# Derek-TH-Wang/OpenRoboRL

Hardware: AMD Instinct MI355X
Metric: env steps/sec at N parallel robots (higher is better)
Workload: dtype f32

## Files before the change

### openroborl_amd/csrc/orr_env_kernels.h

```cpp
#pragma once
#if defined(ORR_PHASE_TIMERS) && !defined(ORR_WAVE_TIMELINE)
#define ORR_WAVE_TIMELINE 1
#endif
#ifndef ORR_TU_MAIN
#undef ORR_PHASE_TIMERS
#endif
#include <hip/hip_runtime.h>
#include <type_traits>
#include <math.h>
#include <stdint.h>
#include <stdio.h>
#include <stdlib.h>
#include <string.h>

#include "orr_device.h"

#ifdef ORR_PHASE_TIMERS
__device__ long long g_phase_cycles[orr::kPhaseSlots];
__device__ long long g_wave_phases[2048 * 40];
#define PT_INIT() do { if (threadIdx.x == 0) { for (int i_ = 0; i_ < orr::kPhaseSlots; i_++) S.pt_acc[i_] = 0; S.pt_last = clock64(); } } while (0)
#define PT(k) do { if (threadIdx.x == 0) { const long long t_ = clock64(); S.pt_acc[k] += t_ - S.pt_last; S.pt_last = clock64(); } } while (0)
#define PT_FLUSH() do { if (threadIdx.x == 0 && blockIdx.x == gridDim.x / 2) for (int i_ = 0; i_ < orr::kPhaseSlots; i_++) atomicAdd((unsigned long long*)&g_phase_cycles[i_], (unsigned long long)S.pt_acc[i_]); \
                        if (threadIdx.x == 0 && blockIdx.x < 2048) for (int i_ = 0; i_ < orr::kPhaseSlots; i_++) g_wave_phases[blockIdx.x * 40 + i_] = S.pt_acc[i_]; } while (0)
#else
// ... 46 lines not shown
  load_robot(P, rec, S, lane);
  const long long total = P.counters[ORR_CNT_TOTAL_STEP_COUNT];
  const ResetConst RC = load_reset_const(P, S, lane);
  float clip_change = 0.0f;
  const uint32_t ep = reset_robot_state<CLIPS, NOISE>(P, S, lane, total, RC, &clip_change, uniforms ? uniforms + (size_t)robot * 28 : nullptr);
  build_obs<NOISE>(P, rec, S, lane, obs, ep, 0u);
  WSYNC();
  store_reset_extras<CLIPS>(rec, S, lane, valid, clip_change);
  store_robot(rec, S, lane, valid);
  if (valid)
    for (int i = lane; i < ORR_OFFEND_ANCHOR_VALID - ORR_OFF_ANCHOR + 1; i += kLanes) rec[O(ANCHOR) + i] = 0.0f;
  if (obs_out && valid)
    for (int i = lane; i < ORR_OBS_DIM; i += kLanes) obs_out[(size_t)robot * ORR_OBS_DIM + i] = obs[i];
}

template <bool CLIPS = true>
__global__ __launch_bounds__(64) void orr_sensor_reset_kernel(KParams P, const uint8_t* mask, float* obs_out, const float* uniforms) {
  ORR_PROLOGUE();
  const bool valid = in_range && !(mask && !mask[robot]);
  load_robot(P, rec, S, lane);
  const long long total = P.counters[ORR_CNT_TOTAL_STEP_COUNT];
  const ResetConst RC = load_reset_const(P, S, lane);
  const SensorNoise SN = load_sensor_noise(P);
  float clip_change = 0.0f;
  const uint32_t ep = reset_robot_state<CLIPS, true, true>(P, S, lane, total, RC, &clip_change, uniforms ? uniforms + (size_t)robot * 28 : nullptr, SN);
  build_obs<true, true>(P, rec, S, lane, obs, ep, 0u, SN);
  WSYNC();
  store_reset_extras<CLIPS>(rec, S, lane, valid, clip_change);
  store_robot(rec, S, lane, valid);
  if (valid)
    for (int i = lane; i < ORR_OFFEND_ANCHOR_VALID - ORR_OFF_ANCHOR + 1; i += kLanes) rec[O(ANCHOR) + i] = 0.0f;
  if (obs_out && valid)
    for (int i = lane; i < ORR_OBS_DIM; i += kLanes) obs_out[(size_t)robot * ORR_OBS_DIM + i] = obs[i];
}

template <bool CLIPS = true>
__global__ __launch_bounds__(64) void orr_randomizer_reset_kernel(KParams P, const uint8_t* mask, float* obs_out, const float* uniforms) {
  ORR_PROLOGUE();
  const bool valid = in_range && !(mask && !mask[robot]);
  load_robot(P, rec, S, lane);
  const long long total = P.counters[ORR_CNT_TOTAL_STEP_COUNT];
  const ResetConst RC = load_reset_const(P, S, lane);
  const SensorNoise SN = load_sensor_noise(P);
  RandRow RR = load_rand_row(P, robot);
  float clip_change = 0.0f;
  const uint32_t ep = reset_robot_state<CLIPS, true, true, true>(P, S, lane, total, RC, &clip_change, uniforms ? uniforms + (size_t)robot * 28 : nullptr, SN, &RR);
  build_obs<true, true>(P, rec, S, lane, obs, ep, 0u, SN);
  WSYNC();
  store_reset_extras<CLIPS>(rec, S, lane, valid, clip_change);
  store_rand_row(P, RR, lane, valid);
  store_robot(rec, S, lane, valid);
  if (valid)
    for (int i = lane; i < ORR_OFFEND_ANCHOR_VALID - ORR_OFF_ANCHOR + 1; i += kLanes) rec[O(ANCHOR) + i] = 0.0f;
  if (obs_out && valid)
    for (int i = lane; i < ORR_OBS_DIM; i += kLanes) obs_out[(size_t)robot * ORR_OBS_DIM + i] = obs[i];
}

#ifndef ORR_WAVES_PER_EU
#define ORR_WAVES_PER_EU 1
#endif
template <int MODE, int WPE = ORR_WAVES_PER_EU, bool ANCHOR = false, bool CLIPS = false, bool NOISE = false>
__global__ __launch_bounds__(64) __attribute__((amdgpu_waves_per_eu(WPE, WPE))) void orr_step_kernel(KParams P, const float* actions, float* obs_out, float* reward_out,
                                                      uint8_t* done_out, int nsub, ReplayArgs RP) {
  constexpr bool TERMS = (MODE & kModeTerms) != 0;
  static_assert(!TERMS || (MODE & 3) != 1, "the debug physics computes no reward");
  constexpr bool CONTACTS = (MODE & kModeContacts) != 0;
  static_assert(!CONTACTS || (MODE & 3) != 2, "the parity replay replaces the physics by recorded states: it has no impulses");
  constexpr bool ACT = (MODE & kModeActuator) != 0;
  static_assert(!ACT || (MODE & 3) != 1, "the debug physics takes its torques as given");
  static_assert(!ACT || TERMS, "the actuator variants are supersets: instantiated with the reward terms only");
  constexpr bool SENS = (MODE & kModeSensor) != 0;
  static_assert(!SENS || (ACT && NOISE), "the sensor variants are supersets: instantiated on top of the actuator variants only");
  constexpr bool RAND = (MODE & kModeRandomizer) != 0;
  static_assert(!RAND || SENS, "the randomiser variants are supersets: instantiated on top of the sensor variants only");
  constexpr bool PUSH = (MODE & kModePush) != 0;
  static_assert(!PUSH || RAND, "the push variant is a superset: instantiated on top of the randomiser variant only");
  static_assert(!PUSH || (MODE & 3) == 0, "the parity replay replaces the physics by recorded states, the debug physics has no env step: neither is pushed");
  ORR_PROLOGUE();
  const bool valid = in_range;
  const orr_config& c = P.cfg;
  PT_INIT();
  WT_INIT();
  const long long total_snapshot = P.counters[ORR_CNT_TOTAL_STEP_COUNT];
  load_robot(P, rec, S, lane);
  bool terms_bound = true, contacts_bound = true, act_bound = false;
  if constexpr (ACT) {
    terms_bound = P.tab->terms != nullptr;
    contacts_bound = P.tab->contact_out != nullptr;
    act_bound = P.tab->act_out != nullptr;
  }
  RandRow RR;
  if constexpr (RAND) RR = load_rand_row(P, robot);
  typedef float __attribute__((address_space(1)))* gpush;
  PushSet PS;
  float push_old = 0.0f, push_w = 0.0f;
  if constexpr (PUSH) {
    PS = load_push(P);
    if (PS.out) push_old = ((gpush)PS.out)[(size_t)robot * ORR_PUSH_ROW + 7];
  }
  float clip_change = 0.0f;
  if constexpr (CLIPS) clip_change = rec[O(CLIP_CHANGE_TIME)];
  {
    static_assert(kHead > ORR_OFF_RING, "spare LDS word behind the state head (the head = everything in front of the ring)");
    bool bad_in = false;
    for (int i = lane; i < 37; i += kLanes) bad_in = bad_in || !(fabsf(S.s[O(POS) + i]) < 1e30f);
    const bool any_bad = ((__ballot(bad_in) >> (sub * kLanes)) & ((1ull << (kLanes - 1)) * 2ull - 1ull)) != 0ull;
    if (lane == 0) S.s[kHead - 1] = any_bad ? 1.0f : 0.0f;
  }
  for (int i = lane; i < kMaxRows * kWStride; i += kLanes) (&S.ph.sub.W[0][0])[i] = 0.0f;
  WSYNC();
  LegConst K;
  load_leg_const(P, S, lane, K);
  {
    float rel[4], Rb[9];
    base_rotation(S, lane, rel, Rb);
  }
  AnchorState AS = {{0.0f, 0.0f, 0.0f}, {0.0f, 0.0f, 0.0f}, 0};
  bool anchor_robot = false;
  const int aleg = lane < 4 ? lane : (lane < 8 ? lane - 4 : (lane - 8) >> 1);
  if constexpr (ANCHOR) {
    static_assert(kLanes == 16, "ANCHOR: aleg indexes the record's four cached points by the 16-lane row layout");
    anchor_robot = model_cold(P, geti(S, O(ROBOT_TYPE)))->friction_anchor != 0;
    const float* an = rec + O(ANCHOR) + 6 * aleg;
    AS.la[0] = an[0]; AS.la[1] = an[1]; AS.la[2] = an[2]; AS.wb[0] = an[3]; AS.wb[1] = an[4]; AS.wb[2] = an[5];
    AS.valid = anchor_robot ? __float_as_int(rec[O(ANCHOR_VALID) + aleg]) : 0;
  }
  auto store_anchor = [&]() __attribute__((always_inline)) {
    if constexpr (ANCHOR) {
      if (valid && lane >= 4 && lane < 8) {
        float* an = rec + O(ANCHOR) + 6 * aleg;
        an[0] = AS.la[0]; an[1] = AS.la[1]; an[2] = AS.la[2]; an[3] = AS.wb[0]; an[4] = AS.wb[1]; an[5] = AS.wb[2];
        rec[O(ANCHOR_VALID) + aleg] = __int_as_float(AS.valid);
      }
    }
  };
  typedef float __attribute__((address_space(1)))* gcontact;
  const int cw = lane < 12 ? lane : 0;
  float c_sum = 0.0f, c_max = 0.0f;
  auto accumulate_contacts = [&]() __attribute__((always_inline)) {
    if constexpr (CONTACTS) {
      const float lw = S.s[O(LAMBDA) + cw];
      c_sum += lw;
      c_max = fmaxf(c_max, lw);
    }
  };
  auto store_contacts = [&]() __attribute__((always_inline)) {
    if constexpr (CONTACTS) {
      if (valid && lane < 12 && contacts_bound) {
        const int cleg = lane / 3, cd = lane - 3 * cleg;
        gcontact const row = (gcontact)P.tab->contact_out + (size_t)robot * 16 + 4 * cleg;
        row[cd] = c_sum;
        if (cd == 0) row[3] = c_max;
      }
    }
  };
  PT(0);

  if ((MODE & 3) == 1) {
    if (lane < 12) {
      const ColdPtr mc = model_cold(P, geti(S, O(ROBOT_TYPE)));
      const int j = mc->joint_of_motor[lane];
      S.tau[j] = mc->tau_sign_motor[lane] * actions[(size_t)robot * 12 + lane];
    }
    WSYNC();
    int fall = 0;
    OwnCoord X;
    load_own_coord(S, lane, X);
    int limit_idle = 0;
    for (int s = 0; s < nsub; s++) {
      fall = physics_substep<ANCHOR>(P, S, K, lane, sub, true, X, limit_idle, ANCHOR ? &AS : nullptr, anchor_robot);
      accumulate_contacts();
      float rel[4], Rb[9];
      base_rotation(S, lane, rel, Rb);
      WSYNC();
    }
    if (valid && lane == 0 && done_out) done_out[robot] = (uint8_t)fall;
    store_robot(rec, S, lane, valid);
    store_anchor();
    store_contacts();
    return;
  }

  const int ml = lane < 12 ? lane : 0;
  const ColdPtr mc = model_cold(P, geti(S, O(ROBOT_TYPE)));
  const int mj = mc->joint_of_motor[ml];
  const float m_off = mc->motor_offset[ml], m_dir = mc->motor_dir[ml], m_kp = mc->kp[ml], m_kd = mc->kd[ml];
  const float m_tsign = mc->tau_sign_motor[ml], m_init = mc->init_motor_angles[ml];
  typedef float __attribute__((address_space(1)))* gact;
  float a_lim = INFINITY, a_tau = 0.0f, a_s1 = 0.0f, a_pk = 0.0f, a_s2 = 0.0f, a_w = 0.0f;
  if constexpr (ACT) a_lim = ((const float __attribute__((address_space(1)))*)&P.tab->torque_limit[geti(S, O(ROBOT_TYPE))][0])[ml];
  SensorNoise SN;
  uint32_t sn_robot = 0u, sn_ep = 0u, sn_i = 0u;
  if constexpr (SENS) {
    SN = load_sensor_noise(P);
    sn_robot = (uint32_t)geti(S, O(ROBOT_INDEX)); sn_ep = (uint32_t)geti(S, O(EPISODE_IDX)); sn_i = 1u + (uint32_t)geti(S, O(EP_STEP));
  }
  ctrl_obs(P, rec, S, lane);
  float act_in = actions[(size_t)robot * 12 + ml];
  {
    const bool bad_act = !(fabsf(act_in) < 1e30f);
    if (bad_act) act_in = 0.0f;
    const bool any_bad = ((__ballot(bad_act) >> (sub * kLanes)) & ((1ull << (kLanes - 1)) * 2ull - 1ull)) != 0ull;
    if (lane == 0 && any_bad) S.s[kHead - 1] = 1.0f;
  }
  if (lane < 12) {
    const float act = act_in + m_init;
    S.s[O(LAST_ACTION) + lane] = act;
    float x1 = S.s[O(XHIST) + lane], x2 = S.s[O(XHIST) + 12 + lane], y1 = S.s[O(YHIST) + lane], y2 = S.s[O(YHIST) + 12 + lane];
    if (geti(S, O(STATE_ACTION_COUNTER)) == 0) {
      float d = map_pi(S.co[lane]);
      if constexpr (SENS) {
        if (SN.a > 0.0f) {
          float u4[4], z0, z1;
          philox_block(c.seed, sn_robot, sn_ep, sensor_block(sn_i, kSensorSlotFilter, (uint32_t)lane), u4);
          normal_pair(u4[0], u4[1], &z0, &z1);
          d = map_pi(fmaf(SN.a, z0, S.co[lane]));
        }
      }
      x1 = x2 = y1 = y2 = d;
    }
    const float y = act * P.fb[0] + (x1 * P.fb[1] + x2 * P.fb[2]) - (y1 * P.fa[1] + y2 * P.fa[2]);
    S.s[O(XHIST) + 12 + lane] = x1; S.s[O(XHIST) + lane] = act;
    S.s[O(YHIST) + 12 + lane] = y1; S.s[O(YHIST) + lane] = y;
    S.s[O(ACTION) + lane] = y;
  }
  if constexpr (PUSH) {
    static_assert(ORR_OFF_ANGVEL == ORR_OFF_LINVEL + 3, "LINVEL and ANGVEL are six consecutive words");
    const uint32_t ps = sn_i - 1u;
    float ua[4], ub[4] = {0.5f, 0.5f, 0.5f, 0.5f};
    philox_block(c.seed, sn_robot, sn_ep, kPushBlock + 2u * ps, ua);
    const bool kicked = (int)ps >= PS.grace && ua[0] < PS.prob;
    float sn, cs;
    unit_sincos(ua[1], &sn, &cs);
    const float pm = fmaf(ua[2], PS.span, PS.lin_lo);
    if (PS.ang > 0.0f) philox_block(c.seed, sn_robot, sn_ep, kPushBlock + 2u * ps + 1u, ub);
    const float two_ang = PS.ang > 0.0f ? 2.0f * PS.ang : 0.0f;
    const float mine = lane == 0 ? __fmul_rn(pm, cs) : (lane == 1 ? __fmul_rn(pm, sn) : (lane == 2 ? fmaf(ua[3], 2.0f * PS.lin_z, -PS.lin_z)
                       : fmaf(lane == 3 ? ub[0] : (lane == 4 ? ub[1] : ub[2]), two_ang, -PS.ang)));
    const float dk = kicked && lane < 6 ? mine : 0.0f;
    if (lane < 6) {
      const float v = S.s[O(LINVEL) + lane];
      S.s[O(LINVEL) + lane] = kicked ? __fadd_rn(v, dk) : v;
    }
    const float one = kicked ? 1.0f : 0.0f;
    push_w = lane < 6 ? dk : (lane == 6 ? one : (ps == 0u ? 0.0f : push_old) + one);
  }
  WSYNC();
  PT(1);
  int fall = 0;
  const float inv_repeat = 1.0f / (float)c.action_repeat;
  const RingLatency rlat = ring_latency(P, S);
  const float m_gain = m_tsign * S.s[O(STRENGTH) + ml];
  const float m_target = S.s[O(ACTION) + ml], m_prev = S.s[O(FILTER_ACTION) + ml];
  const bool m_has_prev = geti(S, O(FILTER_VALID)) != 0;
  int action_counter = geti(S, O(STATE_ACTION_COUNTER));
  RingCursor ring = {geti(S, O(RING_HEAD)), geti(S, O(RING_LEN))};
  OwnCoord X;
  load_own_coord(S, lane, X);
  int limit_idle = 0;
  const int prio_phase = WPE == 2 ? (int)(((unsigned)wave_id / (unsigned)(P.simds > 0 ? P.simds : 1)) & 1u) : 0;
  const bool prio_turns = WPE == 2 && ((((unsigned)gridDim.x + (unsigned)(P.simds > 0 ? P.simds : 1) - 1u) /
                                        (unsigned)(P.simds > 0 ? P.simds : 1)) & 1u) == 0u;
  float co_own = S.co[ml], qm_c = (S.s[O(Q) + mj] - m_off) * m_dir, qdm_c = S.s[O(QD) + mj] * m_dir;
  const uint32_t sn_blk = sensor_block(sn_i, 0u, (uint32_t)ml);
  float sn_u2 = 0.0f, sn_u3 = 0.0f;
  for (int sstep = 0; sstep < c.action_repeat; sstep++) {
    constexpr int kPrioTurn = 4, kPrioHi = 1, kPrioOffset = 1, kPrioEqualFrom = 1000;
    if (WPE == 2 && prio_turns) { if (sstep < kPrioEqualFrom && ((((sstep + kPrioOffset) / kPrioTurn) ^ prio_phase) & 1)) __builtin_amdgcn_s_setprio(kPrioHi); else __builtin_amdgcn_s_setprio(0); }
    {
      const float lerp = (float)(sstep + 1) * inv_repeat;
      float cur = map_pi(co_own), cur_lerp = cur;
      if constexpr (SENS) {
        if (SN.a > 0.0f) {
          float ua, ub, z0, z1;
          if ((sstep & 1) == 0) {
            float u4[4];
            philox_block(c.seed, sn_robot, sn_ep, sn_blk + ((uint32_t)(sstep >> 1) << 4), u4);
            ua = u4[0]; ub = u4[1]; sn_u2 = u4[2]; sn_u3 = u4[3];
          } else {
            ua = sn_u2; ub = sn_u3;
          }
          normal_pair(ua, ub, &z0, &z1);
          cur = map_pi(fmaf(SN.a, z0, co_own));
          cur_lerp = map_pi(fmaf(SN.a, z1, co_own));
        }
      }
      const float prev = m_has_prev ? m_prev : cur_lerp;
      float cmd = prev + lerp * (m_target - prev);
      cmd = fminf(fmaxf(cmd, cur - c.max_angle_change), cur + c.max_angle_change);
      float tq = m_gain * (-1.0f * (m_kp * (qm_c - cmd)) - m_kd * qdm_c);
      if constexpr (ACT) {
        tq = tq > a_lim ? a_lim : (tq < -a_lim ? -a_lim : tq);
        a_tau = tq * m_tsign;
        a_s1 += a_tau;
        a_pk = fmaxf(a_pk, fabsf(a_tau));
        a_s2 = fmaf(a_tau, a_tau, a_s2);
      }
      S.tau[lane < 12 ? mj : lane] = tq;
    }
    WSYNC();
    action_counter++;
    PT(2);
    {
      RingFetch F;
      ring_prefetch(rlat, rec, ring, lane, F);
      if constexpr ((MODE & 3) == 2) {
        const size_t slot = (size_t)robot * c.action_repeat + sstep;
        if (lane < 12 && valid) RP.tau_out[slot * 12 + lane] = S.tau[mj] * m_tsign;
        WSYNC();
        for (int i = lane; i < 37; i += kLanes) S.s[O(POS) + i] = RP.traj[slot * 37 + i];
        WSYNC();
        fall = RP.fall[robot];
      } else
      fall = physics_substep<ANCHOR>(P, S, K, lane, sub, sstep == c.action_repeat - 1, X, limit_idle, ANCHOR ? &AS : nullptr, anchor_robot);
      accumulate_contacts();
      qm_c = (S.s[O(Q) + mj] - m_off) * m_dir;
      qdm_c = S.s[O(QD) + mj] * m_dir;
      if constexpr (ACT) a_w = fmaf(a_tau, qdm_c, a_w);
      ring_push_and_ctrl_obs(rec, S, lane, valid, F, ring, qm_c, &co_own);
    }
    PT(10);
  }
  if (WPE == 2) __builtin_amdgcn_s_setprio(3);
  const ResetConst RC = load_reset_const(P, S, lane);
  float* push_out = nullptr;
  bool push_table = false;
  if constexpr (PUSH) load_push_end(P, &push_out, &push_table);
  if (lane == 0) {
    seti(S, O(RING_HEAD), ring.head); seti(S, O(RING_LEN), ring.len);
    seti(S, O(STATE_ACTION_COUNTER), action_counter);
    seti(S, O(FILTER_VALID), 1);
    seti(S, O(STEP_COUNTER), geti(S, O(STEP_COUNTER)) + 1);
  }
  if (lane < 12) S.s[O(FILTER_ACTION) + lane] = m_target;
  WSYNC();
  if constexpr (SENS) sensors_push_noisy(S, lane, false, SN, c.seed, sn_ep, sn_i);
  else sensors_push(S, lane, false);
  PT(11);
  const DevClip& clip = S.clip;
// ... 446 lines not shown
```

### openroborl_amd/csrc/orr_physics.h

```cpp
#pragma once


__device__ __forceinline__ void chol6(const float A[36], float L[21], float invdiag[6]) {
#pragma unroll
  for (int i = 0; i < 6; i++) {
#pragma unroll
    for (int j = 0; j <= i; j++) {
      float s = A[i * 6 + j];
#pragma unroll
      for (int k = 0; k < j; k++) s -= L[i * (i + 1) / 2 + k] * L[j * (j + 1) / 2 + k];
      if (i == j) {
        const float rs = rsq(s);
        L[i * (i + 1) / 2 + j] = s * rs;
        invdiag[i] = rs;
      } else {
        L[i * (i + 1) / 2 + j] = s * invdiag[j];
      }
    }
  }
}
__device__ __forceinline__ void chol6_solve(const float L[21], const float invdiag[6], const float b[6], float x[6]) {
  float y[6];
#pragma unroll
  for (int i = 0; i < 6; i++) {
// ... 21 lines not shown
  float idg[6];
};
__device__ __forceinline__ void chol6_pk(float d0, float d1, float d3, float d5, float a10, pk2 d2a, pk2 d4a,
                                         pk2 a0a, pk2 a0b, pk2 a1a, pk2 a1b, pk2 a2b, pk2 a3b, Chol6Pk& F) {
  const float r0 = rsq(d0);
  const float l10 = a10 * r0;
  const pk2 c0a = a0a * r0, c0b = a0b * r0;
  d1 = fmaf(-l10, l10, d1);
  a1a = pk_nfma(c0a, l10, a1a); a1b = pk_nfma(c0b, l10, a1b);
  d2a = pk_nfma(c0a, c0a.x, d2a);
  d3 = fmaf(-c0a.y, c0a.y, d3);
  a2b = pk_nfma(c0b, c0a.x, a2b); a3b = pk_nfma(c0b, c0a.y, a3b);
  d4a = pk_nfma(c0b, c0b.x, d4a);
  d5 = fmaf(-c0b.y, c0b.y, d5);
  const float r1 = rsq(d1);
  const pk2 c1a = a1a * r1, c1b = a1b * r1;
  d2a = pk_nfma(c1a, c1a.x, d2a);
  d3 = fmaf(-c1a.y, c1a.y, d3);
  a2b = pk_nfma(c1b, c1a.x, a2b); a3b = pk_nfma(c1b, c1a.y, a3b);
  d4a = pk_nfma(c1b, c1b.x, d4a);
  d5 = fmaf(-c1b.y, c1b.y, d5);
  const float r2 = rsq(d2a.x);
  const float l32 = d2a.y * r2;
  const pk2 c2b = a2b * r2;
  d3 = fmaf(-l32, l32, d3);
  a3b = pk_nfma(c2b, l32, a3b);
  d4a = pk_nfma(c2b, c2b.x, d4a);
  d5 = fmaf(-c2b.y, c2b.y, d5);
  const float r3 = rsq(d3);
  const pk2 c3b = a3b * r3;
  d4a = pk_nfma(c3b, c3b.x, d4a);
  d5 = fmaf(-c3b.y, c3b.y, d5);
  const float r4 = rsq(d4a.x);
  const float l54 = d4a.y * r4;
  d5 = fmaf(-l54, l54, d5);
  F.idg[0] = r0; F.idg[1] = r1; F.idg[2] = r2; F.idg[3] = r3; F.idg[4] = r4; F.idg[5] = rsq(d5);
  F.l10 = l10; F.l32 = l32; F.l54 = l54;
  F.c0a = c0a; F.c0b = c0b; F.c1a = c1a; F.c1b = c1b; F.c2b = c2b; F.c3b = c3b;
}
__device__ __forceinline__ void chol6_solve_pk(const Chol6Pk& F, float b0, float b1, pk2 b23, pk2 b45, float x[6]) {
  float y[6];
  y[0] = b0 * F.idg[0];
  b1 = fmaf(-F.l10, y[0], b1); b23 = pk_nfma(F.c0a, y[0], b23); b45 = pk_nfma(F.c0b, y[0], b45);
  y[1] = b1 * F.idg[1];
  b23 = pk_nfma(F.c1a, y[1], b23); b45 = pk_nfma(F.c1b, y[1], b45);
  y[2] = b23.x * F.idg[2];
  b23.y = fmaf(-F.l32, y[2], b23.y); b45 = pk_nfma(F.c2b, y[2], b45);
  y[3] = b23.y * F.idg[3];
  b45 = pk_nfma(F.c3b, y[3], b45);
  y[4] = b45.x * F.idg[4];
  b45.y = fmaf(-F.l54, y[4], b45.y);
  y[5] = b45.y * F.idg[5];
  x[5] = y[5] * F.idg[5];
  x[4] = fmaf(-F.l54, x[5], y[4]) * F.idg[4];
  x[3] = fmaf(-F.c3b.y, x[5], fmaf(-F.c3b.x, x[4], y[3])) * F.idg[3];
  x[2] = fmaf(-F.c2b.y, x[5], fmaf(-F.c2b.x, x[4], fmaf(-F.l32, x[3], y[2]))) * F.idg[2];
  x[1] = fmaf(-F.c1b.y, x[5], fmaf(-F.c1b.x, x[4], fmaf(-F.c1a.y, x[3], fmaf(-F.c1a.x, x[2], y[1])))) * F.idg[1];
  x[0] = fmaf(-F.c0b.y, x[5], fmaf(-F.c0b.x, x[4], fmaf(-F.c0a.y, x[3], fmaf(-F.c0a.x, x[2], fmaf(-F.l10, x[1], y[0]))))) * F.idg[0];
}

#ifdef ORR_TU_STEP_W2
constexpr bool kCarrySubtreeMass = false, kOwnLegFactor = false, kPackedVelocityUpdate = false;
#define ORR_COMMON(x) (x)
#define ORR_RARE(x) (x)
#else
constexpr bool kCarrySubtreeMass = true, kOwnLegFactor = true, kPackedVelocityUpdate = true;
#define ORR_COMMON(x) __builtin_expect(!!(x), 1)
#define ORR_RARE(x) __builtin_expect(!!(x), 0)
#endif
struct LegConst {
  float r[3][3], jdir[3], joff[3];
  float com[3], m, Ic[6];
  float msub;
  float damp_l, damp_a;
  float jdir_own, joff_own;
  float int_c0, int_c1;
};
struct OwnCoord { float x0, x1; };
__device__ __forceinline__ void load_own_coord(const Shared& S, int lane, OwnCoord& X) {
  X.x0 = lane < 3 ? 0.0f : (lane < 6 ? S.s[O(POS) + lane - 3] : S.s[O(Q) + lane - 6]);
  X.x1 = lane < 2 ? S.s[O(Q) + 10 + lane] : 0.0f;
}
__device__ __forceinline__ float part_suffix_sum(float x);
__device__ static void load_leg_const(const KParams& P, const Shared& S, int lane, LegConst& K) {
  const int leg = lane & 3, part = (lane >> 2) & 3, own = 3 * leg + (part < 3 ? part : 2);
  const ColdPtr mc = model_cold(P, geti(S, O(ROBOT_TYPE)));
#pragma unroll
  for (int k = 0; k < 3; k++) {
    const int j = 3 * leg + k;
    const bool on = k <= part && part < 3;
#pragma unroll
    for (int i = 0; i < 3; i++) K.r[k][i] = on ? S.m.joint_pos[j][i] : 0.0f;
    K.jdir[k] = on ? S.m.jdir[j] : 0.0f;
    K.joff[k] = S.m.joff[j];
  }
  const bool real = part < 3, base = lane == 12;
  const int body = real ? own + 1 : 0;
#pragma unroll
  for (int i = 0; i < 3; i++) K.com[i] = real ? mc->link_com[own][i] : 0.0f;
  {
    const int g = mc->group[body];
    const float mr = S.s[O(MASS_RATIO) + g], ir = S.s[O(INERTIA_RATIO) + g];
    const float mass = mc->mass[body] * mr;
#pragma unroll
    for (int i = 0; i < 6; i++) K.Ic[i] = (real || base) ? mc->inertia[body][i] * ir + mc->inertia_pa[body][i] * mr : 0.0f;
    K.m = (real || base) ? mass : 0.0f;
    if (kCarrySubtreeMass) K.msub = part_suffix_sum(K.m);
  }
  K.jdir_own = real ? S.m.jdir[own] : 0.0f;
  K.joff_own = S.m.joff[own];
  K.damp_l = base ? S.s[O(BASE_DAMPING)] : 0.0f;
  K.damp_a = base ? S.s[O(BASE_DAMPING) + 1] : 0.0f;
  K.int_c0 = lane < 3 ? 0.0f : (lane < 6 ? 1.0f : S.m.jdir[lane < 6 ? 0 : lane - 6]);
  K.int_c1 = lane < 2 ? S.m.jdir[10 + lane] : 0.0f;
}


__device__ __forceinline__ void rot_sym_full(const float R[9], const float S[6], float O[6]) {
  float T[9];
#pragma unroll
  for (int i = 0; i < 3; i++) {
    T[3 * i] = R[3 * i] * S[0] + R[3 * i + 1] * S[3] + R[3 * i + 2] * S[4];
    T[3 * i + 1] = R[3 * i] * S[3] + R[3 * i + 1] * S[1] + R[3 * i + 2] * S[5];
    T[3 * i + 2] = R[3 * i] * S[4] + R[3 * i + 1] * S[5] + R[3 * i + 2] * S[2];
  }
  O[0] = T[0] * R[0] + T[1] * R[1] + T[2] * R[2];
  O[1] = T[3] * R[3] + T[4] * R[4] + T[5] * R[5];
  O[2] = T[6] * R[6] + T[7] * R[7] + T[8] * R[8];
  O[3] = T[0] * R[3] + T[1] * R[4] + T[2] * R[5];
  O[4] = T[0] * R[6] + T[1] * R[7] + T[2] * R[8];
  O[5] = T[3] * R[6] + T[4] * R[7] + T[5] * R[8];
}
__device__ __forceinline__ void spatial_inertia_mul(const float I[6], const float h[3], float m, const float w[3], const float v[3],
                                                    float oa[3], float ol[3]) {
  oa[0] = fmaf(I[0], w[0], fmaf(I[3], w[1], fmaf(I[4], w[2], fmaf(h[1], v[2], -h[2] * v[1]))));
  oa[1] = fmaf(I[3], w[0], fmaf(I[1], w[1], fmaf(I[5], w[2], fmaf(h[2], v[0], -h[0] * v[2]))));
  oa[2] = fmaf(I[4], w[0], fmaf(I[5], w[1], fmaf(I[2], w[2], fmaf(h[0], v[1], -h[1] * v[0]))));
  ol[0] = fmaf(m, v[0], fmaf(h[2], w[1], -h[1] * w[2]));
  ol[1] = fmaf(m, v[1], fmaf(h[0], w[2], -h[2] * w[0]));
  ol[2] = fmaf(m, v[2], fmaf(h[1], w[0], -h[0] * w[1]));
}

template <int AX, bool SAME_AXIS = false>
__device__ __forceinline__ void joint_down(const Shared& S, const LegConst& K, int k, int j, float sn, float cs, float Rw[9], float d[3],
                                           float Vw[3], float Vv[3], float Aa[3], float Al[3], float s[3], float sv[3], float& ad_out,
                                           float* c0 = nullptr) {
  const float ad = K.jdir[k] * S.s[O(QD) + j];
  ad_out = ad;
#pragma unroll
  for (int i = 0; i < 3; i++)
    d[i] = fmaf(Rw[3 * i], K.r[k][0], fmaf(Rw[3 * i + 1], K.r[k][1], fmaf(Rw[3 * i + 2], K.r[k][2], d[i])));
#pragma unroll
  for (int i = 0; i < 3; i++) {
    const float p0 = Rw[3 * i], p1 = Rw[3 * i + 1], p2 = Rw[3 * i + 2];
    if (AX == 0) { Rw[3 * i + 1] = cs * p1 + sn * p2; Rw[3 * i + 2] = -sn * p1 + cs * p2; }
    else { Rw[3 * i] = cs * p0 - sn * p2; Rw[3 * i + 2] = sn * p0 + cs * p2; }
  }
  s[0] = Rw[AX]; s[1] = Rw[3 + AX]; s[2] = Rw[6 + AX];
  cross3(d, s, sv);
  {
    float c0x, c0y, c0z;
    if (SAME_AXIS) { c0x = c0[0]; c0y = c0[1]; c0z = c0[2]; }
    else { c0x = Vw[1] * s[2] - Vw[2] * s[1]; c0y = Vw[2] * s[0] - Vw[0] * s[2]; c0z = Vw[0] * s[1] - Vw[1] * s[0]; }
    if (c0) { c0[0] = c0x; c0[1] = c0y; c0[2] = c0z; }
    const float c1x = fmaf(Vv[1], s[2], fmaf(-Vv[2], s[1], Vw[1] * sv[2] - Vw[2] * sv[1]));
    const float c1y = fmaf(Vv[2], s[0], fmaf(-Vv[0], s[2], Vw[2] * sv[0] - Vw[0] * sv[2]));
    const float c1z = fmaf(Vv[0], s[1], fmaf(-Vv[1], s[0], Vw[0] * sv[1] - Vw[1] * sv[0]));
    Aa[0] = fmaf(ad, c0x, Aa[0]); Aa[1] = fmaf(ad, c0y, Aa[1]); Aa[2] = fmaf(ad, c0z, Aa[2]);
    Al[0] = fmaf(ad, c1x, Al[0]); Al[1] = fmaf(ad, c1y, Al[1]); Al[2] = fmaf(ad, c1z, Al[2]);
#pragma unroll
    for (int i = 0; i < 3; i++) { Vw[i] = fmaf(ad, s[i], Vw[i]); Vv[i] = fmaf(ad, sv[i], Vv[i]); }
  }
}

__device__ __forceinline__ float part_suffix_sum(float x) {
  const int v = __float_as_int(x);
  const float a = __int_as_float(__builtin_amdgcn_update_dpp(0, v, 0x104, 0xF, 0xB, true));
  const float b = __int_as_float(__builtin_amdgcn_update_dpp(0, v, 0x108, 0xF, 0xD, true));
  return x + a + b;
}
#define ORR_SUBTREE_ADD(x, shl, bank) "v_add_f32_dpp " x ", " x ", " x " row_shl:" shl " row_mask:0xf bank_mask:" bank " bound_ctrl:0\n\t"
#define ORR_H_ADD(t, h, shl, bank) "v_add_f32_dpp " t ", " h ", " t " row_shl:" shl " row_mask:0xf bank_mask:" bank " bound_ctrl:0\n\t"
template <bool WITH_M>
__device__ __forceinline__ void part_suffix_sum_first_moment(float& m, const float (&c)[3], float (&h)[3]) {
  static_assert(kRPW == 4, "a robot is one DPP row: lane = leg + 4 part, part = DPP bank");
  float t0, t1, t2;
  if constexpr (WITH_M) {
    asm("v_mov_b32 %0, 0\n\tv_mov_b32 %1, 0\n\tv_mov_b32 %2, 0\n\t"
        ORR_H_ADD("%0", "%4", "4", "0xb") ORR_H_ADD("%1", "%5", "4", "0xb") ORR_H_ADD("%2", "%6", "4", "0xb")
        "v_fmac_f32 %0, %3, %7\n\tv_fmac_f32 %1, %3, %8\n\tv_fmac_f32 %2, %3, %9\n\t"
        ORR_SUBTREE_ADD("%3", "4", "0xb")
        ORR_H_ADD("%0", "%4", "8", "0xd") ORR_H_ADD("%1", "%5", "8", "0xd") ORR_H_ADD("%2", "%6", "8", "0xd")
        ORR_SUBTREE_ADD("%3", "8", "0xd")
        : "=&v"(t0), "=&v"(t1), "=&v"(t2), "+v"(m)
        : "v"(h[0]), "v"(h[1]), "v"(h[2]), "v"(c[0]), "v"(c[1]), "v"(c[2]));
  } else {
    asm("v_mov_b32 %0, 0\n\tv_mov_b32 %1, 0\n\tv_mov_b32 %2, 0\n\t"
// ... 837 lines not shown
```

### openroborl_amd/csrc/orr_robot_io.h

```cpp
#pragma once

typedef float f4 __attribute__((ext_vector_type(4)));
__device__ static void load_robot(const KParams& P, const float* rec, Shared& S, int lane) {
  {
    static_assert(kHead % 4 == 0 && ORR_STATE_STRIDE % 4 == 0, "16-byte pieces");
    typedef const f4 __attribute__((address_space(1))) * g4ptr;
    const g4ptr src = (g4ptr)reinterpret_cast<const f4*>(rec);
    f4* dst = reinterpret_cast<f4*>(S.s);
    constexpr int kQ = kHead / 4, kIt = (kQ + kLanes - 1) / kLanes;
    f4 tmp[kIt];
#pragma unroll
    for (int k = 0; k < kIt; k++) { const int q = lane + k * kLanes; tmp[k] = src[q < kQ ? q : kQ - 1]; }
#pragma unroll
    for (int k = 0; k < kIt; k++) { const int q = lane + k * kLanes; if (q < kQ) dst[q] = tmp[k]; }
  }
  WSYNC();
  const DevModel& gm = P.tab->model[geti(S, O(ROBOT_TYPE))];
  {
    static_assert(sizeof(DevClip) % 4 == 0 && sizeof(DevClip) / 4 <= kLanes, "one word of the clip header per lane");
    const unsigned int* cg = reinterpret_cast<const unsigned int*>(&P.tab->clip[geti(S, O(CLIP_ID))]);
    unsigned int* cl = reinterpret_cast<unsigned int*>(&S.clip);
    if (lane < (int)(sizeof(DevClip) / 4)) cl[lane] = cg[lane];
  }
  {
    typedef const f4 __attribute__((address_space(1))) * g4ptr;
    static_assert(sizeof(ModelHot) % (16 * kLanes) == 0 && alignof(DevModel) >= 16, "whole 16-byte rows of the hot model per lane");
    const g4ptr mp = (g4ptr)reinterpret_cast<const f4*>(&gm.hot);
    f4* dst = reinterpret_cast<f4*>(&S.m);
    constexpr int kIter = (int)(sizeof(ModelHot) / 16) / kLanes;
    f4 tmp[kIter];
#pragma unroll
    for (int k = 0; k < kIter; k++) tmp[k] = mp[lane + k * kLanes];
#pragma unroll
    for (int k = 0; k < kIter; k++) dst[lane + k * kLanes] = tmp[k];
  }
  WSYNC();
}

__device__ static void store_robot(float* rec, const Shared& S, int lane, bool valid) {
  if (valid) {
    typedef f4 __attribute__((address_space(1))) * g4ptr;
    const g4ptr dst = (g4ptr)reinterpret_cast<f4*>(rec);
    const f4* src = reinterpret_cast<const f4*>(S.s);
    constexpr int kQ = O(RING) / 4;
#pragma unroll
    for (int k = 0; k < (kQ + kLanes - 1) / kLanes; k++) { const int q = lane + k * kLanes; if (q < kQ) dst[q] = src[q]; }
    if (lane < O(RING) - 4 * kQ) rec[4 * kQ + lane] = S.s[4 * kQ + lane];
  }
}

__device__ static void ctrl_obs(const KParams& P, const float* rec, Shared& S, int lane) {
  const float lat = S.s[O(LATENCY)], dt = P.cfg.sim_dt;
  const int len = geti(S, O(RING_LEN)), head = geti(S, O(RING_HEAD));
  int k0 = 0, k1 = 0;
  float al = 0.0f;
  if (!(lat <= 0.0f || len == 1)) {
    int n = (int)(lat / dt);
    if (n + 1 >= len) { k0 = k1 = len - 1; }
    else { k0 = n; k1 = n + 1; al = (lat - n * dt) / dt; }
  }
  const int i0 = (head - k0 + 2 * ORR_RING_DEPTH) % ORR_RING_DEPTH, i1 = (head - k1 + 2 * ORR_RING_DEPTH) % ORR_RING_DEPTH;
  for (int i = lane; i < 19; i += kLanes) {
    float e0 = rec[O(RING) + i0 * ORR_RING_ENTRY + i], e1 = rec[O(RING) + i1 * ORR_RING_ENTRY + i];
    S.co[i] = (k0 == k1) ? e0 : (1.0f - al) * e0 + al * e1;
  }
  WSYNC();
}

__device__ __forceinline__ void base_rotation(Shared& S, int lane, float rel[4], float Rb[9]) {
  float qi[4];
  qinv(S.m.init_quat, qi);
  qmul(&S.s[O(QUAT)], qi, rel);
  q_to_mat(rel, Rb);
#pragma unroll
  for (int i = 0; i < 9; i++) S.Rb[i] = Rb[i];
}

struct ResetConst {
  int j;
  float off, dir;
  float init;
  float p0;
};
__device__ __forceinline__ ResetConst load_reset_const(const KParams& P, const Shared& S, int lane) {
  const ColdPtr mc = model_cold(P, geti(S, O(ROBOT_TYPE)));
  const int ml = lane < 12 ? lane : 0;
  return ResetConst{mc->joint_of_motor[ml], mc->motor_offset[ml], mc->motor_dir[ml], mc->init_motor_angles[ml], mc->init_pos[lane < 3 ? lane : 0]};
}

__device__ static void receive_obs(Shared& S, int lane, const ResetConst& RC, float* entry) {
  const int head = (geti(S, O(RING_HEAD)) + 1) % ORR_RING_DEPTH, len = geti(S, O(RING_LEN));
  float rel[4], Rb[9], rate[3];
  base_rotation(S, lane, rel, Rb);
  mtv3(Rb, &S.s[O(ANGVEL)], rate);
  for (int i = lane; i < ORR_RING_ENTRY; i += kLanes) {
    float val = 0.0f;
    if (i < 12) {
      static_assert(kLanes >= 12, "the first pass of the loop covers the twelve motors");
      val = (S.s[O(Q) + RC.j] - RC.off) * RC.dir;
    } else if (i < 16) {
      val = i == 12 ? rel[0] : (i == 13 ? rel[1] : (i == 14 ? rel[2] : rel[3]));
    } else if (i < 19) {
      val = i == 16 ? rate[0] : (i == 17 ? rate[1] : rate[2]);
    }
    entry[i] = val;
  }
  WSYNC();
  if (lane == 0) {
    seti(S, O(RING_HEAD), head);
    seti(S, O(RING_LEN), len + 1 > ORR_RING_DEPTH ? ORR_RING_DEPTH : len + 1);
  }
  WSYNC();
}
__device__ __forceinline__ void store_ring_entry(float* rec, int lane, bool valid, int head, const float* entry) {
  static_assert(ORR_RING_ENTRY == 20 && kLanes == 16, "lane mapping of an entry's words");
  if (valid) {
    float* dst = rec + O(RING) + head * ORR_RING_ENTRY;
    dst[lane] = entry[lane];
    if (lane < 4) dst[16 + lane] = entry[16 + lane];
  }
}

struct RingFetch {
  float e0[2], e1[2];
  float al;
  bool new0, new1, same;
};
struct RingLatency {
  int n;
  float al;
  bool none;
};
__device__ __forceinline__ RingLatency ring_latency(const KParams& P, const Shared& S) {
  const float lat = S.s[O(LATENCY)], dt = P.cfg.sim_dt;
  RingLatency L;
  L.none = lat <= 0.0f;
  L.n = (int)(lat / dt);
  L.al = (lat - L.n * dt) / dt;
  return L;
}
struct RingCursor { int head, len; };
__device__ __forceinline__ int ring_wrap_up(int i) { return i >= ORR_RING_DEPTH ? i - ORR_RING_DEPTH : i; }
__device__ __forceinline__ int ring_wrap_down(int i) { return i < 0 ? i + ORR_RING_DEPTH : i; }
__device__ __forceinline__ void ring_prefetch(const RingLatency& L, const float* rec, const RingCursor& C, int lane, RingFetch& F) {
  const int head = ring_wrap_up(C.head + 1);
  const int len = C.len + 1 > ORR_RING_DEPTH ? ORR_RING_DEPTH : C.len + 1;
  int k0 = 0, k1 = 0;
  F.al = 0.0f;
  if (!(L.none || len == 1)) {
    if (L.n + 1 >= len) { k0 = k1 = len - 1; }
    else { k0 = L.n; k1 = L.n + 1; F.al = L.al; }
  }
  F.same = k0 == k1; F.new0 = k0 == 0; F.new1 = k1 == 0;
  const int i0 = ring_wrap_down(head - k0), i1 = ring_wrap_down(head - k1);
  const float* p0 = rec + O(RING) + i0 * ORR_RING_ENTRY;
  const float* p1 = rec + O(RING) + i1 * ORR_RING_ENTRY;
  const int hi = lane < 3 ? 16 + lane : lane;
  F.e0[0] = p0[lane]; F.e0[1] = p0[hi];
  F.e1[0] = p1[lane]; F.e1[1] = p1[hi];
}
__device__ __forceinline__ void ring_push_and_ctrl_obs(float* rec, Shared& S, int lane, bool valid, const RingFetch& F, RingCursor& C,
                                                       float mang, float* co_own = nullptr) {
  static_assert(ORR_RING_ENTRY == 20, "lane mapping below assumes 20-word entries");
  C.head = ring_wrap_up(C.head + 1);
  C.len = C.len + 1 > ORR_RING_DEPTH ? ORR_RING_DEPTH : C.len + 1;
  float rel[4], Rb[9], rate[3];
  base_rotation(S, lane, rel, Rb);
  mtv3(Rb, &S.s[O(ANGVEL)], rate);
  const float va = lane < 12 ? mang : pick4(lane, rel[0], rel[1], rel[2], rel[3]);
  const float vb = pick4(lane, rate[0], rate[1], rate[2], 0.0f);
  const float a0 = F.new0 ? va : F.e0[0], a1 = F.new1 ? va : F.e1[0];
  const float b0 = F.new0 ? vb : F.e0[1], b1 = F.new1 ? vb : F.e1[1];
  const float co_a = F.same ? a0 : (1.0f - F.al) * a0 + F.al * a1;
  S.co[lane] = co_a;
  if (co_own) *co_own = co_a;
  S.co[lane < 3 ? 16 + lane : 19] = F.same ? b0 : (1.0f - F.al) * b0 + F.al * b1;
  WSYNC();
  float* dst = rec + O(RING) + C.head * ORR_RING_ENTRY;
  if (valid) {
    dst[lane] = va;
    dst[lane < 4 ? 16 + lane : lane] = lane < 4 ? vb : va;
  }
}
```

Measured before the change: 22.15 million.

## Issue all prologue global loads up front before staging into LDS

Splits the robot prologue into issue and stage phases. A few early scalar words (robot type, clip id, ring head/len, latency) are read straight from global memory, so the state head, the hot model, the clip header, the ring observation entries, leg constants, motor constants and actions can all be requested together instead of behind dependent loads and wave syncs. The W zeroing is vectorised to 16-byte stores and placed in the latency shadow. This raises register pressure, since many loads are held in flight at once.

```diff
diff --git a/openroborl_amd/csrc/orr_env_kernels.h b/openroborl_amd/csrc/orr_env_kernels.h
--- a/openroborl_amd/csrc/orr_env_kernels.h
+++ b/openroborl_amd/csrc/orr_env_kernels.h
@@ -152,7 +152,26 @@
   PT_INIT();
   WT_INIT();
   const long long total_snapshot = P.counters[ORR_CNT_TOTAL_STEP_COUNT];
-  load_robot(P, rec, S, lane);
+  const EarlyWords E = load_early_words(rec);
+  HeadLoads HL;
+  head_issue(rec, lane, HL);
+  const RingLatency rlat = ring_latency(P, E.lat);
+  CtrlObsLoads CO;
+  if constexpr ((MODE & 3) != 1) ctrl_obs_issue(rlat, rec, lane, E.head, E.len, CO);
+  ModelLoads ML;
+  model_issue(P, E.type, E.clip, lane, ML);
+  LegColdLoads KL;
+  leg_const_issue(P, E.type, lane, KL);
+  const int ml = lane < 12 ? lane : 0;
+  const ColdPtr mc = model_cold(P, E.type);
+  const int mj = mc->joint_of_motor[ml];
+  const float m_off = mc->motor_offset[ml], m_dir = mc->motor_dir[ml], m_kp = mc->kp[ml], m_kd = mc->kd[ml];
+  const float m_tsign = mc->tau_sign_motor[ml], m_init = mc->init_motor_angles[ml];
+  typedef float __attribute__((address_space(1)))* gact;
+  float a_lim = INFINITY;
+  if constexpr (ACT) a_lim = ((const float __attribute__((address_space(1)))*)&P.tab->torque_limit[E.type][0])[ml];
+  float act_in = 0.0f;
+  if constexpr ((MODE & 3) != 1) act_in = actions[(size_t)robot * 12 + ml];
   bool terms_bound = true, contacts_bound = true, act_bound = false;
   if constexpr (ACT) {
     terms_bound = P.tab->terms != nullptr;
@@ -171,16 +190,28 @@
   float clip_change = 0.0f;
   if constexpr (CLIPS) clip_change = rec[O(CLIP_CHANGE_TIME)];
   {
+    static_assert((kMaxRows * kWStride) % 4 == 0, "whole 16-byte pieces");
+    constexpr int kW4 = kMaxRows * kWStride / 4;
+    f4* w4 = reinterpret_cast<f4*>(&S.ph.sub.W[0][0]);
+    const f4 zero4 = {0.0f, 0.0f, 0.0f, 0.0f};
+#pragma unroll
+    for (int k = 0; k < (kW4 + kLanes - 1) / kLanes; k++) { const int q = lane + k * kLanes; w4[q < kW4 ? q : kW4 - 1] = zero4; }
+  }
+  const float inv_repeat = 1.0f / (float)c.action_repeat;
+  head_stage(S, lane, HL);
+  if constexpr ((MODE & 3) != 1) ctrl_obs_finish(S, lane, CO);
+  model_stage(S, lane, ML);
+  WSYNC();
+  {
     static_assert(kHead > ORR_OFF_RING, "spare LDS word behind the state head (the head = everything in front of the ring)");
     bool bad_in = false;
     for (int i = lane; i < 37; i += kLanes) bad_in = bad_in || !(fabsf(S.s[O(POS) + i]) < 1e30f);
     const bool any_bad = ((__ballot(bad_in) >> (sub * kLanes)) & ((1ull << (kLanes - 1)) * 2ull - 1ull)) != 0ull;
     if (lane == 0) S.s[kHead - 1] = any_bad ? 1.0f : 0.0f;
   }
-  for (int i = lane; i < kMaxRows * kWStride; i += kLanes) (&S.ph.sub.W[0][0])[i] = 0.0f;
   WSYNC();
   LegConst K;
-  load_leg_const(P, S, lane, K);
+  load_leg_const(S, lane, KL, K);
   {
     float rel[4], Rb[9];
     base_rotation(S, lane, rel, Rb);
@@ -190,7 +221,7 @@
   const int aleg = lane < 4 ? lane : (lane < 8 ? lane - 4 : (lane - 8) >> 1);
   if constexpr (ANCHOR) {
     static_assert(kLanes == 16, "ANCHOR: aleg indexes the record's four cached points by the 16-lane row layout");
-    anchor_robot = model_cold(P, geti(S, O(ROBOT_TYPE)))->friction_anchor != 0;
+    anchor_robot = mc->friction_anchor != 0;
     const float* an = rec + O(ANCHOR) + 6 * aleg;
     AS.la[0] = an[0]; AS.la[1] = an[1]; AS.la[2] = an[2]; AS.wb[0] = an[3]; AS.wb[1] = an[4]; AS.wb[2] = an[5];
     AS.valid = anchor_robot ? __float_as_int(rec[O(ANCHOR_VALID) + aleg]) : 0;
@@ -227,11 +258,7 @@
   PT(0);
 
   if ((MODE & 3) == 1) {
-    if (lane < 12) {
-      const ColdPtr mc = model_cold(P, geti(S, O(ROBOT_TYPE)));
-      const int j = mc->joint_of_motor[lane];
-      S.tau[j] = mc->tau_sign_motor[lane] * actions[(size_t)robot * 12 + lane];
-    }
+    if (lane < 12) S.tau[mj] = m_tsign * actions[(size_t)robot * 12 + lane];
     WSYNC();
     int fall = 0;
     OwnCoord X;
@@ -251,22 +278,13 @@
     return;
   }
 
-  const int ml = lane < 12 ? lane : 0;
-  const ColdPtr mc = model_cold(P, geti(S, O(ROBOT_TYPE)));
-  const int mj = mc->joint_of_motor[ml];
-  const float m_off = mc->motor_offset[ml], m_dir = mc->motor_dir[ml], m_kp = mc->kp[ml], m_kd = mc->kd[ml];
-  const float m_tsign = mc->tau_sign_motor[ml], m_init = mc->init_motor_angles[ml];
-  typedef float __attribute__((address_space(1)))* gact;
-  float a_lim = INFINITY, a_tau = 0.0f, a_s1 = 0.0f, a_pk = 0.0f, a_s2 = 0.0f, a_w = 0.0f;
-  if constexpr (ACT) a_lim = ((const float __attribute__((address_space(1)))*)&P.tab->torque_limit[geti(S, O(ROBOT_TYPE))][0])[ml];
+  float a_tau = 0.0f, a_s1 = 0.0f, a_pk = 0.0f, a_s2 = 0.0f, a_w = 0.0f;
   SensorNoise SN;
   uint32_t sn_robot = 0u, sn_ep = 0u, sn_i = 0u;
   if constexpr (SENS) {
     SN = load_sensor_noise(P);
     sn_robot = (uint32_t)geti(S, O(ROBOT_INDEX)); sn_ep = (uint32_t)geti(S, O(EPISODE_IDX)); sn_i = 1u + (uint32_t)geti(S, O(EP_STEP));
   }
-  ctrl_obs(P, rec, S, lane);
-  float act_in = actions[(size_t)robot * 12 + ml];
   {
     const bool bad_act = !(fabsf(act_in) < 1e30f);
     if (bad_act) act_in = 0.0f;
@@ -318,13 +336,11 @@
   WSYNC();
   PT(1);
   int fall = 0;
-  const float inv_repeat = 1.0f / (float)c.action_repeat;
-  const RingLatency rlat = ring_latency(P, S);
   const float m_gain = m_tsign * S.s[O(STRENGTH) + ml];
   const float m_target = S.s[O(ACTION) + ml], m_prev = S.s[O(FILTER_ACTION) + ml];
   const bool m_has_prev = geti(S, O(FILTER_VALID)) != 0;
   int action_counter = geti(S, O(STATE_ACTION_COUNTER));
-  RingCursor ring = {geti(S, O(RING_HEAD)), geti(S, O(RING_LEN))};
+  RingCursor ring = {E.head, E.len};
   OwnCoord X;
   load_own_coord(S, lane, X);
   int limit_idle = 0;
diff --git a/openroborl_amd/csrc/orr_physics.h b/openroborl_amd/csrc/orr_physics.h
--- a/openroborl_amd/csrc/orr_physics.h
+++ b/openroborl_amd/csrc/orr_physics.h
@@ -127,9 +127,20 @@
   X.x1 = lane < 2 ? S.s[O(Q) + 10 + lane] : 0.0f;
 }
 __device__ __forceinline__ float part_suffix_sum(float x);
-__device__ static void load_leg_const(const KParams& P, const Shared& S, int lane, LegConst& K) {
+struct LegColdLoads { float com[3], mass, inertia[6], inertia_pa[6]; int group; };
+__device__ __forceinline__ void leg_const_issue(const KParams& P, int robot_type, int lane, LegColdLoads& L) {
   const int leg = lane & 3, part = (lane >> 2) & 3, own = 3 * leg + (part < 3 ? part : 2);
-  const ColdPtr mc = model_cold(P, geti(S, O(ROBOT_TYPE)));
+  const int body = part < 3 ? own + 1 : 0;
+  const ColdPtr mc = model_cold(P, robot_type);
+#pragma unroll
+  for (int i = 0; i < 3; i++) L.com[i] = mc->link_com[own][i];
+  L.group = mc->group[body];
+  L.mass = mc->mass[body];
+#pragma unroll
+  for (int i = 0; i < 6; i++) { L.inertia[i] = mc->inertia[body][i]; L.inertia_pa[i] = mc->inertia_pa[body][i]; }
+}
+__device__ static void load_leg_const(const Shared& S, int lane, const LegColdLoads& L, LegConst& K) {
+  const int leg = lane & 3, part = (lane >> 2) & 3, own = 3 * leg + (part < 3 ? part : 2);
 #pragma unroll
   for (int k = 0; k < 3; k++) {
     const int j = 3 * leg + k;
@@ -140,15 +151,14 @@
     K.joff[k] = S.m.joff[j];
   }
   const bool real = part < 3, base = lane == 12;
-  const int body = real ? own + 1 : 0;
-#pragma unroll
-  for (int i = 0; i < 3; i++) K.com[i] = real ? mc->link_com[own][i] : 0.0f;
-  {
-    const int g = mc->group[body];
+#pragma unroll
+  for (int i = 0; i < 3; i++) K.com[i] = real ? L.com[i] : 0.0f;
+  {
+    const int g = L.group;
     const float mr = S.s[O(MASS_RATIO) + g], ir = S.s[O(INERTIA_RATIO) + g];
-    const float mass = mc->mass[body] * mr;
-#pragma unroll
-    for (int i = 0; i < 6; i++) K.Ic[i] = (real || base) ? mc->inertia[body][i] * ir + mc->inertia_pa[body][i] * mr : 0.0f;
+    const float mass = L.mass * mr;
+#pragma unroll
+    for (int i = 0; i < 6; i++) K.Ic[i] = (real || base) ? fmaf(L.inertia[i], ir, L.inertia_pa[i] * mr) : 0.0f;
     K.m = (real || base) ? mass : 0.0f;
     if (kCarrySubtreeMass) K.msub = part_suffix_sum(K.m);
   }
@@ -158,6 +168,11 @@
   K.damp_a = base ? S.s[O(BASE_DAMPING) + 1] : 0.0f;
   K.int_c0 = lane < 3 ? 0.0f : (lane < 6 ? 1.0f : S.m.jdir[lane < 6 ? 0 : lane - 6]);
   K.int_c1 = lane < 2 ? S.m.jdir[10 + lane] : 0.0f;
+}
+__device__ __forceinline__ void load_leg_const(const KParams& P, const Shared& S, int lane, LegConst& K) {
+  LegColdLoads L;
+  leg_const_issue(P, geti(S, O(ROBOT_TYPE)), lane, L);
+  load_leg_const(S, lane, L, K);
 }
 
 
diff --git a/openroborl_amd/csrc/orr_robot_io.h b/openroborl_amd/csrc/orr_robot_io.h
--- a/openroborl_amd/csrc/orr_robot_io.h
+++ b/openroborl_amd/csrc/orr_robot_io.h
@@ -1,40 +1,60 @@
 #pragma once
 
 typedef float f4 __attribute__((ext_vector_type(4)));
+struct HeadLoads { f4 q[(kHead / 4 + kLanes - 1) / kLanes]; };
+struct ModelLoads { f4 q[(int)(sizeof(ModelHot) / 16) / kLanes]; unsigned int clip; };
+__device__ __forceinline__ void head_issue(const float* rec, int lane, HeadLoads& H) {
+  static_assert(kHead % 4 == 0 && ORR_STATE_STRIDE % 4 == 0, "16-byte pieces");
+  typedef const f4 __attribute__((address_space(1))) * g4ptr;
+  const g4ptr src = (g4ptr)reinterpret_cast<const f4*>(rec);
+  constexpr int kQ = kHead / 4, kIt = (kQ + kLanes - 1) / kLanes;
+#pragma unroll
+  for (int k = 0; k < kIt; k++) { const int q = lane + k * kLanes; H.q[k] = src[q < kQ ? q : kQ - 1]; }
+}
+__device__ __forceinline__ void head_stage(Shared& S, int lane, const HeadLoads& H) {
+  f4* dst = reinterpret_cast<f4*>(S.s);
+  constexpr int kQ = kHead / 4, kIt = (kQ + kLanes - 1) / kLanes;
+#pragma unroll
+  for (int k = 0; k < kIt; k++) { const int q = lane + k * kLanes; if (q < kQ) dst[q] = H.q[k]; }
+}
+__device__ __forceinline__ void model_issue(const KParams& P, int robot_type, int clip_id, int lane, ModelLoads& M) {
+  typedef const f4 __attribute__((address_space(1))) * g4ptr;
+  typedef const unsigned int __attribute__((address_space(1))) * guptr;
+  static_assert(sizeof(ModelHot) % (16 * kLanes) == 0 && alignof(DevModel) >= 16, "whole 16-byte rows of the hot model per lane");
+  static_assert(sizeof(DevClip) / 4 == kLanes, "one word of the clip header per lane");
+  const g4ptr mp = (g4ptr)reinterpret_cast<const f4*>(&P.tab->model[robot_type].hot);
+  constexpr int kIter = (int)(sizeof(ModelHot) / 16) / kLanes;
+#pragma unroll
+  for (int k = 0; k < kIter; k++) M.q[k] = mp[lane + k * kLanes];
+  M.clip = ((guptr)reinterpret_cast<const unsigned int*>(&P.tab->clip[clip_id]))[lane];
+}
+__device__ __forceinline__ void model_stage(Shared& S, int lane, const ModelLoads& M) {
+  f4* dst = reinterpret_cast<f4*>(&S.m);
+  constexpr int kIter = (int)(sizeof(ModelHot) / 16) / kLanes;
+#pragma unroll
+  for (int k = 0; k < kIter; k++) dst[lane + k * kLanes] = M.q[k];
+  reinterpret_cast<unsigned int*>(&S.clip)[lane] = M.clip;
+}
 __device__ static void load_robot(const KParams& P, const float* rec, Shared& S, int lane) {
-  {
-    static_assert(kHead % 4 == 0 && ORR_STATE_STRIDE % 4 == 0, "16-byte pieces");
-    typedef const f4 __attribute__((address_space(1))) * g4ptr;
-    const g4ptr src = (g4ptr)reinterpret_cast<const f4*>(rec);
-    f4* dst = reinterpret_cast<f4*>(S.s);
-    constexpr int kQ = kHead / 4, kIt = (kQ + kLanes - 1) / kLanes;
-    f4 tmp[kIt];
-#pragma unroll
-    for (int k = 0; k < kIt; k++) { const int q = lane + k * kLanes; tmp[k] = src[q < kQ ? q : kQ - 1]; }
-#pragma unroll
-    for (int k = 0; k < kIt; k++) { const int q = lane + k * kLanes; if (q < kQ) dst[q] = tmp[k]; }
-  }
-  WSYNC();
-  const DevModel& gm = P.tab->model[geti(S, O(ROBOT_TYPE))];
-  {
-    static_assert(sizeof(DevClip) % 4 == 0 && sizeof(DevClip) / 4 <= kLanes, "one word of the clip header per lane");
-    const unsigned int* cg = reinterpret_cast<const unsigned int*>(&P.tab->clip[geti(S, O(CLIP_ID))]);
-    unsigned int* cl = reinterpret_cast<unsigned int*>(&S.clip);
-    if (lane < (int)(sizeof(DevClip) / 4)) cl[lane] = cg[lane];
-  }
-  {
-    typedef const f4 __attribute__((address_space(1))) * g4ptr;
-    static_assert(sizeof(ModelHot) % (16 * kLanes) == 0 && alignof(DevModel) >= 16, "whole 16-byte rows of the hot model per lane");
-    const g4ptr mp = (g4ptr)reinterpret_cast<const f4*>(&gm.hot);
-    f4* dst = reinterpret_cast<f4*>(&S.m);
-    constexpr int kIter = (int)(sizeof(ModelHot) / 16) / kLanes;
-    f4 tmp[kIter];
-#pragma unroll
-    for (int k = 0; k < kIter; k++) tmp[k] = mp[lane + k * kLanes];
-#pragma unroll
-    for (int k = 0; k < kIter; k++) dst[lane + k * kLanes] = tmp[k];
-  }
-  WSYNC();
+  HeadLoads H;
+  head_issue(rec, lane, H);
+  head_stage(S, lane, H);
+  WSYNC();
+  ModelLoads M;
+  model_issue(P, geti(S, O(ROBOT_TYPE)), geti(S, O(CLIP_ID)), lane, M);
+  model_stage(S, lane, M);
+  WSYNC();
+}
+
+struct EarlyWords { int type, clip, head, len; float lat; };
+__device__ __forceinline__ EarlyWords load_early_words(const float* rec) {
+  typedef const float __attribute__((address_space(1))) * gfp;
+  const gfp r = (gfp)rec;
+  EarlyWords E;
+  E.type = __float_as_int(r[O(ROBOT_TYPE)]); E.clip = __float_as_int(r[O(CLIP_ID)]);
+  E.head = __float_as_int(r[O(RING_HEAD)]); E.len = __float_as_int(r[O(RING_LEN)]);
+  E.lat = r[O(LATENCY)];
+  return E;
 }
 
 __device__ static void store_robot(float* rec, const Shared& S, int lane, bool valid) {
@@ -49,20 +69,46 @@
   }
 }
 
-__device__ static void ctrl_obs(const KParams& P, const float* rec, Shared& S, int lane) {
-  const float lat = S.s[O(LATENCY)], dt = P.cfg.sim_dt;
-  const int len = geti(S, O(RING_LEN)), head = geti(S, O(RING_HEAD));
+struct RingLatency {
+  int n;
+  float al;
+  bool none;
+};
+__device__ __forceinline__ RingLatency ring_latency(const KParams& P, float lat) {
+  const float dt = P.cfg.sim_dt;
+  RingLatency L;
+  L.none = lat <= 0.0f;
+  L.n = (int)(lat / dt);
+  L.al = (lat - L.n * dt) / dt;
+  return L;
+}
+struct CtrlObsLoads { float e0[2], e1[2], al; bool same; };
+__device__ __forceinline__ int ring_wrap_down(int i);
+__device__ __forceinline__ void ctrl_obs_issue(const RingLatency& L, const float* rec, int lane, int head, int len, CtrlObsLoads& F) {
+  typedef const float __attribute__((address_space(1))) * gfp;
+  static_assert(ORR_RING_ENTRY == 20 && kLanes == 16, "lane mapping of an entry's words");
   int k0 = 0, k1 = 0;
   float al = 0.0f;
-  if (!(lat <= 0.0f || len == 1)) {
-    int n = (int)(lat / dt);
-    if (n + 1 >= len) { k0 = k1 = len - 1; }
-    else { k0 = n; k1 = n + 1; al = (lat - n * dt) / dt; }
-  }
-  const int i0 = (head - k0 + 2 * ORR_RING_DEPTH) % ORR_RING_DEPTH, i1 = (head - k1 + 2 * ORR_RING_DEPTH) % ORR_RING_DEPTH;
-  for (int i = lane; i < 19; i += kLanes) {
-    float e0 = rec[O(RING) + i0 * ORR_RING_ENTRY + i], e1 = rec[O(RING) + i1 * ORR_RING_ENTRY + i];
-    S.co[i] = (k0 == k1) ? e0 : (1.0f - al) * e0 + al * e1;
+  if (!(L.none || len == 1)) {
+    if (L.n + 1 >= len) { k0 = k1 = len - 1; }
+    else { k0 = L.n; k1 = L.n + 1; al = L.al; }
+  }
+  const int i0 = ring_wrap_down(head - k0), i1 = ring_wrap_down(head - k1);
+  const gfp p0 = (gfp)rec + O(RING) + i0 * ORR_RING_ENTRY, p1 = (gfp)rec + O(RING) + i1 * ORR_RING_ENTRY;
+  const int hi = lane < 3 ? 16 + lane : lane;
+  F.e0[0] = p0[lane]; F.e1[0] = p1[lane];
+  F.e0[1] = p0[hi]; F.e1[1] = p1[hi];
+  F.al = al; F.same = k0 == k1;
+}
+__device__ __forceinline__ void ctrl_obs_finish(Shared& S, int lane, const CtrlObsLoads& F) {
+  const float al = F.al;
+  {
+    const float e0 = F.e0[0], e1 = F.e1[0];
+    S.co[lane] = F.same ? e0 : (1.0f - al) * e0 + al * e1;
+  }
+  {
+    const float e0 = F.e0[1], e1 = F.e1[1];
+    S.co[lane < 3 ? 16 + lane : 19] = F.same ? e0 : (1.0f - al) * e0 + al * e1;
   }
   WSYNC();
 }
@@ -126,19 +172,6 @@
   float al;
   bool new0, new1, same;
 };
-struct RingLatency {
-  int n;
-  float al;
-  bool none;
-};
-__device__ __forceinline__ RingLatency ring_latency(const KParams& P, const Shared& S) {
-  const float lat = S.s[O(LATENCY)], dt = P.cfg.sim_dt;
-  RingLatency L;
-  L.none = lat <= 0.0f;
-  L.n = (int)(lat / dt);
-  L.al = (lat - L.n * dt) / dt;
-  return L;
-}
 struct RingCursor { int head, len; };
 __device__ __forceinline__ int ring_wrap_up(int i) { return i >= ORR_RING_DEPTH ? i - ORR_RING_DEPTH : i; }
 __device__ __forceinline__ int ring_wrap_down(int i) { return i < 0 ? i + ORR_RING_DEPTH : i; }
```

Result: no change. 22.17 million, median of 4 (+0.1%).
